# rubengooj/stvo-pl

Hardware: AMD Instinct MI355X
Metric: stereo frames/s (match+optimizePose) (higher is better)
Workload: dtype u8/fp4+f64; 1 GPU; BASELINE configs[2]: KITTI-00-shaped stereo with points + lines (ORB + LBD rows), grid-windowed stereo match (points and lines) + f2f brute-force mutual-NNR match (points and lines) + full GN optimizePose (config_kitti.yaml), device-resident per-frame pipeline; the streams cycle through the 8 sequence ids / 3 KITTI calibrations of configs[4] (sequence s on rank s mod G); streams_per_gpu=3072, parallelism=seq-shard x1

## Files before the change

stvo-pl_amd/csrc/grid_kernels.hip:

```cpp
#include <cstdlib>
#include <vector>

#include "ctx_internal.h"
#include "point_cells.h"

namespace stvo {
namespace {

#ifndef GRID_ROWS_PER_TRIP
#define GRID_ROWS_PER_TRIP 1
#endif
constexpr unsigned long long kTop2Empty = 0x00000000FFFFFFFFull;

struct GridArgs {
    const int32_t* cell_xy1;
    const uint8_t* d1;
    int n1;
    const int32_t* cell_start;
    const int32_t* cell_items;
    const uint8_t* d2;
    int n2;
    const double* dir2;
    stvo_grid_window w;
    double ratio, line_sim_th;
    int mutual;
    int words64;
    int n1p;
    unsigned long long* cover;
    const int32_t* rank;
    const int32_t* perm;
    unsigned long long* top2;
    int32_t* owner2;
    int32_t* m12;
    uint32_t* elig;
    int32_t* elig_cnt;
    int32_t* ovf;
    int elig_stride;
    const int32_t* range1;
};

__device__ __forceinline__ GridArgs frame_view(const GridBatch& g, int b) {
    GridArgs a;
    a.cell_xy1 = g.cell_xy1 + (size_t)b * g.stride1 * g.xy_width;
    a.d1 = g.d1 + (size_t)b * g.stride1 * STVO_DESC_BYTES;
    a.n1 = g.n1[b];
    a.cell_start = g.cell_start + (size_t)b * (STVO_GRID_CELLS + 1);
    a.cell_items = g.cell_items + (size_t)b * g.items_stride;
    a.d2 = g.d2 + (size_t)b * g.stride2 * STVO_DESC_BYTES;
    a.n2 = g.n2[b];
    a.dir2 = g.dir2 ? g.dir2 + (size_t)b * g.stride2 * 2 : nullptr;
    a.w = g.w;
    a.ratio = g.ratio;
    a.line_sim_th = g.line_sim_th;
    a.mutual = g.mutual;
    a.words64 = g.words64;
    a.n1p = g.n1p;
    a.cover = g.cover + (size_t)b * g.words64 * g.n1p;
    a.rank = g.rank + (size_t)b * g.stride2;
    a.perm = g.perm + (size_t)b * g.stride2;
    a.top2 = g.top2 + (size_t)b * g.stride1;
    a.owner2 = g.owner2 + (size_t)b * g.stride2;
    a.m12 = g.m12 + (size_t)b * g.stride1;
    a.elig = g.elig ? g.elig + (size_t)b * GRID_ELIG * g.stride2 : nullptr;
    a.elig_cnt = g.elig ? g.elig_cnt + (size_t)b * g.stride2 : nullptr;
    a.ovf = g.elig ? g.ovf + b : nullptr;
    a.elig_stride = g.stride2;
    a.range1 = g.range1 ? g.range1 + (size_t)b * g.stride1 * 2 : nullptr;
    return a;
}

template <typename P>
__device__ __forceinline__ void cover_window(const GridArgs& a, int x, int y, P col, size_t stride) {
    const int min_x = max(0, x - a.w.w_lo), max_x = min(STVO_GRID_COLS, x + a.w.w_hi + 1);
    const int min_y = max(0, y - a.w.h_lo), max_y = min(STVO_GRID_ROWS, y + a.w.h_hi + 1);
    for (int yy = min_y; yy < max_y; ++yy) {
        if (min_x >= max_x) break;
        const int lo = a.cell_start[yy * STVO_GRID_COLS + min_x], hi = a.cell_start[yy * STVO_GRID_COLS + max_x];
        for (int k = lo; k < hi; ++k) {
            const int id = a.cell_items[k];
            if (id >= 0 && id < a.n2) {
                const int p = a.rank[id];
                col[(size_t)(p >> 6) * stride] |= 1ull << (p & 63);
            }
        }
// ... 220 lines not shown
    }
}

__global__ __launch_bounds__(256) void grid_elig_kernel(GridBatch g) {
    grid_elig_body(frame_view(g, blockIdx.y), blockIdx.x * 256 + threadIdx.x);
}

__device__ __forceinline__ void grid_finalize_body(const GridArgs& a, const int i1, const int stride1) {
    if (i1 >= stride1) return;
    if (i1 >= a.n1) {
        a.m12[i1] = -1;
        return;
    }
    const unsigned long long t = a.top2[i1];
    const uint32_t b = (uint32_t)t, blocked = (uint32_t)(t >> 32);
    int m = -1;
    if (b != 0xFFFFFFFFu && !blocked && (double)(int)(b >> 16) < 2147483647.0 * a.ratio) m = (int)(b & 0xFFFFu);
    if (a.mutual && m >= 0 && a.owner2[m] != i1) m = -1;
    a.m12[i1] = m;
}

__global__ __launch_bounds__(256) void grid_finalize_kernel(GridBatch g) {
    grid_finalize_body(frame_view(g, blockIdx.y), blockIdx.x * 256 + threadIdx.x, g.stride1);
}

constexpr int FUSED_T = 1024, FUSED_ROWS = 2048, FUSED_REG = 16, FUSED_R = FUSED_ROWS / FUSED_T;
constexpr int FUSED_LW = GRID_LW;
constexpr int FUSED_PADDED = FUSED_ROWS + FUSED_REG;
constexpr int FUSED_KEY_CAP = 8192;
constexpr int FUSED_WQ = 256, FUSED_WQ_WORDS = 12;
constexpr size_t FUSED_LDS = (size_t)FUSED_PADDED * (16 + 16 + 2) + (size_t)FUSED_ROWS * (4 + 2 + 2 + 1) + (size_t)FUSED_KEY_CAP * 4 +
                             (size_t)FUSED_WQ * FUSED_WQ_WORDS * 4;

__device__ __forceinline__ void fused_misfit_frame(const GridBatch& g, const int f) {
    const GridArgs a = frame_view(g, f);
    const int stride1 = g.stride1;
    const int tid = threadIdx.x, lane = tid & 63, wave = tid >> 6;
    const int blocks = (a.n2 + 63) >> 6;
    if (g.lean_cells) {
        const int32_t* cs = g.cell_start + (size_t)f * (STVO_GRID_CELLS + 1);
        const uint32_t* ls = g.lstart + (size_t)f * GRID_LSTART_STRIDE;
        const int32_t* lp = g.lperm + (size_t)f * g.stride1;
        int32_t* rg = const_cast<int32_t*>(g.range1) + (size_t)f * g.stride1 * 2;
        for (int i = tid; i < stride1; i += FUSED_T) {
            a.top2[i] = kTop2Empty;
            rg[2 * i] = 0;
            rg[2 * i + 1] = 0;
        }
        if (tid == 0 && a.ovf) *a.ovf = 0;
        __builtin_amdgcn_fence(__ATOMIC_RELEASE, "agent");
        __syncthreads();
        __builtin_amdgcn_fence(__ATOMIC_ACQUIRE, "agent");
        const int n_in = cs[STVO_GRID_CELLS];
        for (int c = tid; c < GRID_LCELLS; c += FUSED_T) {
            const int y = c / GRID_LW, x = c - y * GRID_LW;
            const int min_x = min(max(0, x - g.w.w_lo), STVO_GRID_COLS), max_x = max(min(STVO_GRID_COLS, x + 1), min_x);
            const int c0 = y * STVO_GRID_COLS + min_x, c1 = y * STVO_GRID_COLS + max_x;
            const int lo = c0 < STVO_GRID_CELLS ? cs[c0] : n_in, hi = c1 < STVO_GRID_CELLS ? cs[c1] : n_in;
            for (uint32_t pos = ls[c]; pos < ls[c + 1]; ++pos) {
                const int i1 = lp[pos];
                rg[2 * i1] = lo;
                rg[2 * i1 + 1] = hi;
            }
        }
        __builtin_amdgcn_fence(__ATOMIC_RELEASE, "agent");
        __syncthreads();
        __builtin_amdgcn_fence(__ATOMIC_ACQUIRE, "agent");
    }
    for (int w = wave; w < blocks; w += FUSED_T / 64) grid_scan_body<false, 1, true>(a, w * 64 + lane);
    __builtin_amdgcn_fence(__ATOMIC_RELEASE, "agent");
    __syncthreads();
    __builtin_amdgcn_fence(__ATOMIC_ACQUIRE, "agent");
    if (a.elig)
        for (int w = wave; w < blocks; w += FUSED_T / 64) grid_elig_body(a, w * 64 + lane);
    for (int w = wave; w < blocks; w += FUSED_T / 64) grid_scan_body<false, 2, true>(a, w * 64 + lane);
    __builtin_amdgcn_fence(__ATOMIC_RELEASE, "agent");
    __syncthreads();
    __builtin_amdgcn_fence(__ATOMIC_ACQUIRE, "agent");
    for (int i1 = tid; i1 < stride1; i1 += FUSED_T) grid_finalize_body(a, i1, stride1);
}

typedef uint32_t u32x4 __attribute__((ext_vector_type(4)));
__device__ __forceinline__ uint4 lds_row(const uint4* p) {
    const u32x4 v = *reinterpret_cast<const u32x4*>(p);
    return make_uint4(v.x, v.y, v.z, v.w);
}

__device__ __forceinline__ uint32_t hamming256(const uint4& t0, const uint4& t1, const uint4& q0, const uint4& q1) {
    uint32_t dd = __builtin_popcount(t0.x ^ q0.x);
    dd = bcnt_acc(t0.y ^ q0.y, dd);
    dd = bcnt_acc(t0.z ^ q0.z, dd);
    dd = bcnt_acc(t0.w ^ q0.w, dd);
    dd = bcnt_acc(t1.x ^ q1.x, dd);
    dd = bcnt_acc(t1.y ^ q1.y, dd);
    dd = bcnt_acc(t1.z ^ q1.z, dd);
    dd = bcnt_acc(t1.w ^ q1.w, dd);
    return dd;
}

__device__ __forceinline__ void sort16(uint32_t (&k)[FUSED_REG]) {
#pragma unroll
    for (int size = 2; size <= FUSED_REG; size <<= 1) {
#pragma unroll
        for (int j = size >> 1; j > 0; j >>= 1) {
#pragma unroll
            for (int i = 0; i < FUSED_REG; ++i) {
                const int l = i ^ j;
                if (l > i) {
                    const uint32_t lo = min(k[i], k[l]), hi = max(k[i], k[l]);
                    const bool asc = (i & size) == 0;
                    k[i] = asc ? lo : hi;
                    k[l] = asc ? hi : lo;
                }
            }
        }
    }
}

constexpr int FUSED_EK = 4;
constexpr uint32_t FUSED_NOKEY = 0xFFFFFFFFu, FUSED_FLAG = 1u << 30;

struct FusedNext {
    int i1[FUSED_R], i2[FUSED_R], rc[FUSED_R];
    u32x4 l0[FUSED_R], l1[FUSED_R];
    u32x4 q0[FUSED_R], q1[FUSED_R];
    int la[FUSED_R], lb[FUSED_R];
};

struct FusedHdr {
    int n_placed, n2, n1;
};
__device__ __forceinline__ FusedHdr fused_hdr(const GridBatch& g, const int f) {
    FusedHdr h;
    h.n_placed = (int)g.lstart[(size_t)f * GRID_LSTART_STRIDE + GRID_LCELLS];
    h.n2 = g.n2[f];
    h.n1 = g.n1[f];
    return h;
}

__device__ __forceinline__ int fresh(int v) {
    asm volatile("" : "+v"(v));
    return v;
}

__device__ __forceinline__ void fused_fetch1(const GridBatch& g, const int f, FusedNext& n) {
    const int tid = fresh(threadIdx.x);
    const int32_t* __restrict__ cell2 = g.cell2 + (size_t)f * g.stride2;
    const int32_t* __restrict__ lperm = g.lperm + (size_t)f * g.stride1;
    const int32_t* __restrict__ perm = g.perm + (size_t)f * g.stride2;
#pragma unroll
    for (int r = 0; r < FUSED_R; ++r) {
        const int pos = tid + r * FUSED_T;
        const int p1 = pos < g.stride1 ? pos : g.stride1 - 1, p2 = pos < g.stride2 ? pos : g.stride2 - 1;
        n.i1[r] = lperm[p1];
        n.i2[r] = perm[p2];
        n.rc[r] = cell2[p2];
    }
}

__device__ __forceinline__ void fused_fetch2(const GridBatch& g, const int f, const FusedHdr& h, FusedNext& n) {
    const int tid = fresh(threadIdx.x);
    const u32x4* __restrict__ D1 = reinterpret_cast<const u32x4*>(g.d1) + (size_t)f * g.stride1 * 2;
    const u32x4* __restrict__ D2 = reinterpret_cast<const u32x4*>(g.d2) + (size_t)f * g.stride2 * 2;
    const uint32_t* __restrict__ lstart = g.lstart + (size_t)f * GRID_LSTART_STRIDE;
#pragma unroll
    for (int r = 0; r < FUSED_R; ++r) {
        const int pos = tid + r * FUSED_T;
        const int i1 = pos < h.n_placed ? n.i1[r] : 0, i2 = pos < h.n2 ? n.i2[r] : 0, rc = pos < h.n2 ? n.rc[r] : 0;
        n.l0[r] = D1[2 * i1];
        n.l1[r] = D1[2 * i1 + 1];
        n.q0[r] = D2[2 * i2];
        n.q1[r] = D2[2 * i2 + 1];
        const int y = rc >> 6, x = rc & (STVO_GRID_COLS - 1);
        n.la[r] = (int)lstart[y * FUSED_LW + x];
        n.lb[r] = (int)lstart[y * FUSED_LW + x + g.w.w_lo + 1];
    }
}

__device__ __forceinline__ void fused_tail(const GridBatch& g, const int f, const int n1, const int (&mm)[FUSED_R], int* s_cnt) {
    const PointTail& t = g.tail;
    int tid = threadIdx.x;
    asm volatile("" : "+v"(tid));
    const int lane = tid & 63, wv = tid >> 6;
    const size_t off = (size_t)f * g.stride1;
    bool ok[FUSED_R];
    double disp[FUSED_R];
    int before[FUSED_R];
#pragma unroll
    for (int r = 0; r < FUSED_R; ++r) {
        const int i = tid + r * FUSED_T;
        ok[r] = false;
        disp[r] = 0.0;
        if (i < n1 && mm[r] >= 0) ok[r] = point_tail_filter(t, off, i, mm[r], disp[r]);
        const unsigned long long bal = __ballot(ok[r]);
        before[r] = __popcll(bal & ((1ull << lane) - 1ull));
        if (lane == 0) s_cnt[r * (FUSED_T / 64) + wv] = __popcll(bal);
    }
    __syncthreads();
    int base = 0;
#pragma unroll
    for (int r = 0; r < FUSED_R; ++r) {
        int wbase = base;
        for (int w = 0; w < FUSED_T / 64; ++w) {
            const int c = s_cnt[r * (FUSED_T / 64) + w];
            wbase += w < wv ? c : 0;
            base += c;
        }
        if (ok[r]) point_tail_write(t, off, tid + r * FUSED_T, off + (size_t)(wbase + before[r]), disp[r]);
    }
    if (tid == 0) {
        t.n[f] = base;
        if (t.host_n) t.host_n[f] = base;
        if (t.zero_nl) t.nl[f] = 0;
    }
}

template <bool CELLS>
__global__ __launch_bounds__(FUSED_T) void grid_points_fused_kernel(GridBatch g, const int key_cap) {
    extern __shared__ uint4 s_fused[];
    static_assert(sizeof(PointCellsLds<FUSED_T>) <= FUSED_LDS, "the cells phase borrows the matcher's LDS");
    if (CELLS) {
        if ((int)blockIdx.x >= g.B) return;
        point_cells_frame<FUSED_T, true>(g.cells, blockIdx.x, reinterpret_cast<PointCellsLds<FUSED_T>*>(s_fused));
        __builtin_amdgcn_fence(__ATOMIC_RELEASE, "agent");
        __syncthreads();
        __builtin_amdgcn_fence(__ATOMIC_ACQUIRE, "agent");
    }
    __shared__ int s_cnt[FUSED_R * (FUSED_T / 64)];
    __shared__ int s_ctl[3];
    uint4* s_llo = s_fused;
    uint4* s_lhi = s_llo + FUSED_PADDED;
    uint32_t* s_best = reinterpret_cast<uint32_t*>(s_lhi + FUSED_PADDED);
    uint32_t* s_keys = s_best + FUSED_ROWS;
    unsigned short* s_lperm = reinterpret_cast<unsigned short*>(s_keys + FUSED_KEY_CAP);
    unsigned short* s_owner = s_lperm + FUSED_PADDED;
    unsigned short* s_rperm = s_owner + FUSED_ROWS;
    unsigned char* s_blocked = reinterpret_cast<unsigned char*>(s_rperm + FUSED_ROWS);
    uint32_t* s_wq = reinterpret_cast<uint32_t*>(s_blocked + FUSED_ROWS);
    const int tid = threadIdx.x;
    FusedNext nx;
    int f = blockIdx.x, f_n1 = f + (int)gridDim.x, f_n2 = f + 2 * (int)gridDim.x;
    if (f >= g.B) return;
    unsigned long long misfit_mask = 0ull;
    int trip = 0;
    FusedHdr hn = fused_hdr(g, f);
    fused_fetch1(g, f, nx);
    FusedHdr hc;
    hc.n_placed = __builtin_amdgcn_readfirstlane(hn.n_placed);
    hc.n2 = __builtin_amdgcn_readfirstlane(hn.n2);
    hc.n1 = __builtin_amdgcn_readfirstlane(hn.n1);
    fused_fetch2(g, f, hc, nx);
    if (f_n1 < g.B) hn = fused_hdr(g, f_n1);
    const bool mutual = g.mutual != 0;
    const double ratio = g.ratio;
    FusedHdr hs = hc;
    auto commit_rows = [&](const FusedHdr& h) {
        const int t0 = fresh(tid);
#pragma unroll
        for (int r = 0; r < FUSED_R; ++r) {
            const int pos = t0 + r * FUSED_T;
            if (pos < h.n_placed) {
                *reinterpret_cast<u32x4*>(s_llo + pos) = nx.l0[r];
                *reinterpret_cast<u32x4*>(s_lhi + pos) = nx.l1[r];
                s_lperm[pos] = (unsigned short)nx.i1[r];
            }
        }
        hs.n_placed = __builtin_amdgcn_readfirstlane(hn.n_placed);
        hs.n2 = __builtin_amdgcn_readfirstlane(hn.n2);
        hs.n1 = __builtin_amdgcn_readfirstlane(hn.n1);
    };
    commit_rows(hc);
    for (; f < g.B; f = f_n1, f_n1 = f_n2, f_n2 += (int)gridDim.x) {
        uint4 q0[FUSED_R], q1[FUSED_R];
        int la[FUSED_R], cnt[FUSED_R];
        const int t1 = fresh(tid);
#pragma unroll
        for (int r = 0; r < FUSED_R; ++r) {
            const int pos = t1 + r * FUSED_T;
            if (pos < hc.n2) s_rperm[pos] = (unsigned short)nx.i2[r];
            s_best[pos] = 0xFFFFFFFFu;
            s_blocked[pos] = 0;
            q0[r] = make_uint4(nx.q0[r].x, nx.q0[r].y, nx.q0[r].z, nx.q0[r].w);
            q1[r] = make_uint4(nx.q1[r].x, nx.q1[r].y, nx.q1[r].z, nx.q1[r].w);
            la[r] = pos < hc.n2 ? nx.la[r] : 0;
            cnt[r] = pos < hc.n2 ? nx.lb[r] - nx.la[r] : 0;
        }
        if (tid == 0) {
            s_ctl[0] = 0;
            s_ctl[1] = key_cap < 0;
            s_ctl[2] = 0;
        }
        const int fn = f_n1;
        const bool more = fn < g.B;
        if (more) {
            fused_fetch1(g, fn, nx);
            if (f_n2 < g.B) hn = fused_hdr(g, f_n2);
        }
        __syncthreads();
        uint32_t ek[FUSED_R][FUSED_EK];
        uint32_t kinfo[FUSED_R] = {};
#pragma unroll
        for (int r = 0; r < FUSED_R; ++r) {
            const int p = tid + r * FUSED_T;
            uint32_t key[FUSED_REG];
            uint32_t elig = 0u;
            bool wide = cnt[r] > FUSED_REG;
            if (wide) {
                const int xoff = atomicAdd(&s_ctl[0], cnt[r]);
                const int slot = atomicAdd(&s_ctl[2], 1);
                if (xoff + cnt[r] > key_cap || slot >= FUSED_WQ) {
                    s_ctl[1] = 1;
                    wide = false;
                    cnt[r] = 0;
                } else {
                    kinfo[r] = (uint32_t)cnt[r] | ((uint32_t)xoff << 12) | 0x80000000u;
                    uint32_t* e = s_wq + slot * FUSED_WQ_WORDS;
                    e[0] = (uint32_t)p; e[1] = (uint32_t)la[r]; e[2] = (uint32_t)cnt[r]; e[3] = (uint32_t)xoff;
                    e[4] = q0[r].x; e[5] = q0[r].y; e[6] = q0[r].z; e[7] = q0[r].w;
                    e[8] = q1[r].x; e[9] = q1[r].y; e[10] = q1[r].z; e[11] = q1[r].w;
                }
            }
            const int c16 = wide ? 0 : cnt[r];
            const uint4* lo_row = s_llo + la[r];
            const uint4* hi_row = s_lhi + la[r];
            const unsigned short* perm_row = s_lperm + la[r];
#pragma unroll
            for (int k4 = 0; k4 < FUSED_REG; k4 += 4) {
                if (!__any(c16 > k4)) {
#pragma unroll
                    for (int j = 0; j < 4; ++j) key[k4 + j] = FUSED_NOKEY;
                    continue;
                }
#pragma unroll
                for (int j = 0; j < 4; ++j) {
                    const uint32_t dd = hamming256(lds_row(lo_row + k4 + j), lds_row(hi_row + k4 + j), q0[r], q1[r]);
                    const uint32_t i1 = perm_row[k4 + j];
                    key[k4 + j] = k4 + j < c16 ? ((i1 << 9) | dd) : FUSED_NOKEY;
                }
            }
            uint32_t owner = 0xFFFFu;
            if (mutual) {
                sort16(key);
                uint32_t thr = 512u;
#pragma unroll
                for (int k = 0; k < FUSED_REG; ++k) {
                    const uint32_t dd = key[k] & 511u;
                    if (key[k] != FUSED_NOKEY && dd < thr) {
                        thr = dd;
                        owner = key[k] >> 9;
                        elig |= 1u << k;
                    }
                }
            } else {
                elig = (1u << c16) - 1u;
            }
            int extra = __builtin_popcount(elig) - FUSED_EK, eoff = 0;
            if (extra > 0) {
                eoff = atomicAdd(&s_ctl[0], extra);
                if (eoff + extra > key_cap) {
                    s_ctl[1] = 1;
                    extra = 0;
                } else {
                    kinfo[r] = (uint32_t)extra | ((uint32_t)eoff << 12);
                }
            }
#pragma unroll
            for (int j = 0; j < FUSED_EK; ++j) ek[r][j] = FUSED_NOKEY;
            int ne = 0;
#pragma unroll
            for (int k = 0; k < FUSED_REG; ++k)
                if (elig & (1u << k)) {
                    atomicMin(&s_best[key[k] >> 9], ((key[k] & 511u) << 16) | (uint32_t)p);
#pragma unroll
                    for (int j = 0; j < FUSED_EK; ++j) ek[r][j] = ne == j ? key[k] : ek[r][j];
                    if (k >= FUSED_EK && ne >= FUSED_EK && ne - FUSED_EK < extra) s_keys[eoff + ne - FUSED_EK] = key[k];
                    ++ne;
                }
            if (!wide) s_owner[p] = (unsigned short)owner;
            if (wide && !mutual) s_owner[p] = 0xFFFFu;
        }
        if (more) fused_fetch2(g, fn, hs, nx);
        __syncthreads();
        const bool misfit = s_ctl[1] != 0;
        const int n_wide = s_ctl[2];
        if (!misfit && n_wide > 0) {
            for (int ent = tid >> 6; ent < n_wide; ent += FUSED_T / 64) {
                const uint32_t* e = s_wq + ent * FUSED_WQ_WORDS;
                const uint32_t w_p = (uint32_t)__builtin_amdgcn_readfirstlane((int)e[0]);
                const int w_la = __builtin_amdgcn_readfirstlane((int)e[1]), w_cnt = __builtin_amdgcn_readfirstlane((int)e[2]);
                const int w_xoff = __builtin_amdgcn_readfirstlane((int)e[3]);
                const uint4 wq0 = make_uint4(e[4], e[5], e[6], e[7]), wq1 = make_uint4(e[8], e[9], e[10], e[11]);
                uint32_t* kk = s_keys + w_xoff;
                for (int k = tid & 63; k < w_cnt; k += 64) {
                    const int pos = w_la + k;
                    kk[k] = ((uint32_t)s_lperm[pos] << 9) | hamming256(lds_row(s_llo + pos), lds_row(s_lhi + pos), wq0, wq1);
                }
                __builtin_amdgcn_fence(__ATOMIC_RELEASE, "wavefront");
                __builtin_amdgcn_wave_barrier();
                __builtin_amdgcn_fence(__ATOMIC_ACQUIRE, "wavefront");
                for (int k = tid & 63; k < w_cnt; k += 64) {
                    const uint32_t mine = kk[k] & ~FUSED_FLAG, i1 = mine >> 9, dd = mine & 511u;
                    bool dominated = false, later_better = false;
                    for (int j = 0; j < w_cnt; ++j) {
                        const uint32_t v = kk[j], vi = (v >> 9) & 2047u, vd = v & 511u;
                        dominated |= vi < i1 && vd <= dd;
                        later_better |= vi > i1 && vd < dd;
                    }
                    if (!mutual || !dominated) {
                        kk[k] = mine | FUSED_FLAG;
                        atomicMin(&s_best[i1], (dd << 16) | w_p);
                        if (mutual && !later_better) s_owner[w_p] = (unsigned short)i1;
                    }
                }
            }
            __syncthreads();
        }
        if (tid == 0) g.misfit[f] = misfit;
        if (misfit && trip < 64) misfit_mask |= 1ull << trip;
        ++trip;
        if (!misfit) {
#pragma unroll
            for (int r = 0; r < FUSED_R; ++r) {
                const uint32_t p = (uint32_t)(tid + r * FUSED_T);
                auto judge = [&](uint32_t k, uint32_t pos) {
                    const uint32_t i1 = (k >> 9) & 2047u, dd = k & 511u;
                    const uint32_t bk = s_best[i1];
                    if (bk != ((dd << 16) | pos)) {
                        const double best_d = (double)(int)(bk >> 16), d2 = (double)(int)dd;
                        if (!(best_d < d2 * ratio)) s_blocked[i1] = 1;
                    }
                };
#pragma unroll
                for (int j = 0; j < FUSED_EK; ++j)
                    if (ek[r][j] != FUSED_NOKEY) judge(ek[r][j], p);
                if (!(kinfo[r] >> 31))
                    for (uint32_t j = 0; j < (kinfo[r] & 4095u); ++j) judge(s_keys[((kinfo[r] >> 12) & 0x3FFFFu) + j], p);
                for (unsigned long long wm = __ballot((kinfo[r] >> 31) != 0u); wm; wm &= wm - 1ull) {
                    const int L = __builtin_ctzll(wm);
                    const uint32_t w_info = (uint32_t)__builtin_amdgcn_readlane((int)kinfo[r], L);
                    const int w_cnt = (int)(w_info & 4095u), w_xoff = (int)((w_info >> 12) & 0x3FFFFu);
                    const uint32_t w_p = (uint32_t)((tid & ~63) + L + r * FUSED_T);
                    for (int k = tid & 63; k < w_cnt; k += 64) {
                        const uint32_t v = s_keys[w_xoff + k];
                        if (v & FUSED_FLAG) judge(v & ~FUSED_FLAG, w_p);
                    }
                }
            }
        }
        const FusedHdr hfn = hs;
        if (more) commit_rows(hfn);
        __syncthreads();
        if (!misfit) {
            int mm[FUSED_R];
#pragma unroll
            for (int r = 0; r < FUSED_R; ++r) {
                const int i1 = tid + r * FUSED_T;
                mm[r] = -1;
                if (i1 >= g.stride1) continue;
                const uint32_t bk = s_best[i1];
                if (i1 < hc.n1 && bk != 0xFFFFFFFFu && !s_blocked[i1] && (double)(int)(bk >> 16) < 2147483647.0 * ratio) {
                    const int pb = (int)(bk & 0xFFFFu);
                    if (!mutual || (int)s_owner[pb] == i1) mm[r] = (int)s_rperm[pb];
                }
                g.m12[(size_t)f * g.stride1 + i1] = mm[r];
            }
            if (g.has_tail) fused_tail(g, f, hc.n1, mm, s_cnt);
        }
        if (more) __syncthreads();
        hc = hfn;
    }
    if (misfit_mask != 0ull || trip > 64) {
        int i = 0;
        for (int fm = (int)blockIdx.x; fm < g.B; fm += (int)gridDim.x, ++i) {
            const bool todo = i < 64 ? ((misfit_mask >> i) & 1ull) != 0ull : g.misfit[fm] != 0;
            if (todo) {
                __syncthreads();
                fused_misfit_frame(g, fm);
                if (g.has_tail) {
                    __builtin_amdgcn_fence(__ATOMIC_RELEASE, "agent");
                    __syncthreads();
                    __builtin_amdgcn_fence(__ATOMIC_ACQUIRE, "agent");
                    int mm[FUSED_R];
#pragma unroll
                    for (int r = 0; r < FUSED_R; ++r) {
                        const int i1 = threadIdx.x + r * FUSED_T;
                        mm[r] = i1 < g.stride1 ? g.m12[(size_t)fm * g.stride1 + i1] : -1;
                    }
                    fused_tail(g, fm, g.n1[fm], mm, s_cnt);
                }
            }
        }
    }
}

}

bool grid_points_fused_ok(const GridBatch& g) {
    const bool range = g.range_points && g.range1 != nullptr;
    const bool fused = range && g.misfit && g.cell2 && g.lperm && g.lstart && g.stride1 <= FUSED_ROWS && g.stride2 <= FUSED_ROWS && g.w.w_lo >= 0 &&
                       g.w.w_lo <= FUSED_LW - STVO_GRID_COLS && g.w.w_hi == 0 && g.w.h_lo == 0 && g.w.h_hi == 0 && dbg().grid_fused != 0;
    return fused && lds_opt_in(reinterpret_cast<const void*>(grid_points_fused_kernel<false>), (int)FUSED_LDS) &&
           lds_opt_in(reinterpret_cast<const void*>(grid_points_fused_kernel<true>), (int)FUSED_LDS);
}

void launch_grid_batch(hipStream_t s, const GridBatch& g, bool lines, hipEvent_t* scan_events) {
    if (g.B <= 0 || g.stride1 <= 0 || g.stride2 <= 0) return;
    const dim3 g1((g.stride1 + 255) / 256, g.B), g2((g.stride2 + 255) / 256, g.B), gc((g.n1p + 255) / 256, g.B), blk(256);
    const size_t lds = (size_t)g.words64 * 256 * sizeof(unsigned long long);
    const bool use_lds = lds <= ((size_t)64 << 10);
    if (lines) {
        if (use_lds)
            hipLaunchKernelGGL((grid_cover_kernel<true, true>), gc, blk, lds, s, g);
        else
            hipLaunchKernelGGL((grid_cover_kernel<true, false>), gc, blk, 0, s, g);
        if (scan_events && scan_events[0]) (void)hipEventRecord(scan_events[0], s);
        hipLaunchKernelGGL((grid_scan_kernel<true, 1, false>), g2, blk, 0, s, g);
        if (g.elig) hipLaunchKernelGGL(grid_elig_kernel, g2, blk, 0, s, g);
        hipLaunchKernelGGL((grid_scan_kernel<true, 2, false>), g2, blk, 0, s, g);
        if (scan_events) (void)hipEventRecord(scan_events[1], s);
    } else {
        const bool range = g.range_points && g.range1 != nullptr;
        if (grid_points_fused_ok(g)) {
            int cap = dbg().grid_fused_cap != DBG_UNSET ? dbg().grid_fused_cap : FUSED_KEY_CAP;
            if (cap > FUSED_KEY_CAP) cap = FUSED_KEY_CAP;
            const int fused_wgs = device_cu_count();
            if (scan_events && scan_events[0]) (void)hipEventRecord(scan_events[0], s);
            if (g.fused_cells && g.B <= fused_wgs)
                hipLaunchKernelGGL(grid_points_fused_kernel<true>, dim3(g.B), dim3(FUSED_T), FUSED_LDS, s, g, cap);
            else
                hipLaunchKernelGGL(grid_points_fused_kernel<false>, dim3(g.B < fused_wgs ? g.B : fused_wgs), dim3(FUSED_T), FUSED_LDS, s, g, cap);
            if (scan_events) (void)hipEventRecord(scan_events[1], s);
            return;
        }
        if (range) {
            if (scan_events && scan_events[0]) (void)hipEventRecord(scan_events[0], s);
            hipLaunchKernelGGL((grid_scan_kernel<false, 1, true>), g2, blk, 0, s, g);
            if (g.elig) hipLaunchKernelGGL(grid_elig_kernel, g2, blk, 0, s, g);
            hipLaunchKernelGGL((grid_scan_kernel<false, 2, true>), g2, blk, 0, s, g);
        } else {
            if (use_lds)
                hipLaunchKernelGGL((grid_cover_kernel<false, true>), gc, blk, lds, s, g);
            else
                hipLaunchKernelGGL((grid_cover_kernel<false, false>), gc, blk, 0, s, g);
            if (scan_events && scan_events[0]) (void)hipEventRecord(scan_events[0], s);
            hipLaunchKernelGGL((grid_scan_kernel<false, 1, false>), g2, blk, 0, s, g);
            if (g.elig) hipLaunchKernelGGL(grid_elig_kernel, g2, blk, 0, s, g);
            hipLaunchKernelGGL((grid_scan_kernel<false, 2, false>), g2, blk, 0, s, g);
        }
        if (scan_events) (void)hipEventRecord(scan_events[1], s);
    }
    hipLaunchKernelGGL(grid_finalize_kernel, g1, blk, 0, s, g);
}

void launch_grid_range_debug(hipStream_t s, const GridBatch& g) {
    hipLaunchKernelGGL(grid_range_debug_kernel, dim3((g.n1p + 255) / 256, g.B), dim3(256), 0, s, g);
}

namespace {

template <bool LINES>
int run_grid(stvo_ctx* ctx, const int32_t* cell_xy1, const uint8_t* d1, int n1, const int32_t* cell_start,
             const int32_t* cell_items, const uint8_t* d2, int n2, const double* dir2, const stvo_grid_window* w,
             double ratio, double line_sim_th, int mutual, int32_t* m12, int32_t* n_matches) {
// ... 117 lines not shown
```

stvo-pl_amd/csrc/match_mfma.hip:

```cpp
#include <type_traits>

#include "kernels.h"

namespace stvo {

typedef int v4i __attribute__((ext_vector_type(4)));
typedef int v8i __attribute__((ext_vector_type(8)));
typedef int v16i __attribute__((ext_vector_type(16)));
typedef float v16f __attribute__((ext_vector_type(16)));

#ifndef MF_TPB
#define MF_TPB 2
#endif
#ifndef MF_FOLD_SLOTS
#define MF_FOLD_SLOTS 5
#endif
constexpr int MF_BLOCK = 256;
constexpr int MF_TILE = 32;
constexpr int MF_KEY_SHIFT = 13;
constexpr int MF_KEY_BIAS = 1 << 20;
constexpr int MF_NO_KEY = 0x7FFFFFFF;
constexpr int MF_NO_KEY_MIN = 0x40000000;

__device__ __forceinline__ v4i expand_fp4(uint32_t w) {
    v4i r;
    r.x = (int)(((w << 3) & 0x88888888u) | 0x66666666u);
    r.y = (int)(((w << 2) & 0x88888888u) | 0x66666666u);
    r.z = (int)(((w << 1) & 0x88888888u) | 0x66666666u);
    r.w = (int)((w & 0x88888888u) | 0x66666666u);
    return r;
}
__device__ __forceinline__ float med3_f32(float a, float b, float c) {
    float r;
    asm("v_med3_f32 %0, %1, %2, %3" : "=v"(r) : "v"(a), "v"(b), "v"(c));
    return r;
}
__device__ __forceinline__ float min_f32(float a, float b) {
    float r;
    asm("v_min_f32 %0, %1, %2" : "=v"(r) : "v"(a), "v"(b));
    return r;
}
__device__ __forceinline__ float max_f32(float a, float b) {
    float r;
    asm("v_max_f32 %0, %1, %2" : "=v"(r) : "v"(a), "v"(b));
    return r;
}
__device__ __forceinline__ float min3_f32(float a, float b, float c) {
    float r;
    asm("v_min3_f32 %0, %1, %2, %3" : "=v"(r) : "v"(a), "v"(b), "v"(c));
    return r;
}
constexpr float MF_NO_KEY_F = 1.0e30f;
constexpr float MF_NO_KEY_MIN_F = 1.0e29f;
constexpr int MF_SCALE_2_4 = 127 + 4;

__device__ __forceinline__ uint32_t key_to_knn(int key, int base) {
    if (key >= MF_NO_KEY_MIN) return 0xFFFFFFFFu;
    const uint32_t u = (uint32_t)(key + base + MF_KEY_BIAS);
    return ((u >> MF_KEY_SHIFT) << 16) | (u & ((1u << MF_KEY_SHIFT) - 1u));
}

template <int QB, int MODE>
// ... 461 lines not shown
```

stvo-pl_amd/csrc/point_tail.h:

```cpp
#pragma once

#include <hip/hip_runtime.h>
#include <stdint.h>

#include "../../include/stvo_hip.h"

namespace stvo {

struct PointTail {
    const float* kp_l;
    const float* kp_r;
    const int32_t* oct_l;
    const uint8_t* desc_l;
    const stvo_cam* cams;
    double max_dist_epip, min_disp;
    float4* rc;
    uint8_t* desc;
    int32_t* n;
    int32_t* host_n;
    int32_t* nl;
    int zero_nl;
};

__device__ __forceinline__ bool point_tail_filter(const PointTail& t, size_t off, int i, int i2, double& disp) {
    const float yl = t.kp_l[(off + i) * 2 + 1], yr = t.kp_r[(off + i2) * 2 + 1];
    if (!((double)fabsf(yl - yr) <= t.max_dist_epip)) return false;
    disp = (double)(t.kp_l[(off + i) * 2 + 0] - t.kp_r[(off + i2) * 2 + 0]);
    return disp >= t.min_disp;
}

__device__ __forceinline__ void point_tail_write(const PointTail& t, size_t off, int i, size_t k, double disp) {
    t.rc[k] = make_float4(t.kp_l[(off + i) * 2 + 0], t.kp_l[(off + i) * 2 + 1], (float)disp, (float)t.oct_l[off + i]);
    const uint4* src = reinterpret_cast<const uint4*>(t.desc_l + (off + i) * STVO_DESC_BYTES);
    uint4* dst = reinterpret_cast<uint4*>(t.desc + k * STVO_DESC_BYTES);
    dst[0] = src[0];
    dst[1] = src[1];
}

}
```

Measured before the change: 1.380 million frame-pairs/s.

## Read fused grid kernel args from kernarg segment and tighten inner-loop instructions

The fused point grid matcher now reads GridBatch fields through the kernarg segment pointer on each use instead of holding a by-value copy, aiming to cut scalar register pressure. The Hamming key building folds the i1<<9 term into the popcount accumulator and masks invalid slots with a bit-field sign extract instead of a select. The eligible-key buffering becomes a shift register, and the tail prefetches left keypoints, batches right-keypoint loads and computes disparity in float. The fp4 expansion uses a single and-or instruction, and an optional cycle-counter probe, compiled out by default, is added.

```diff
diff --git a/stvo-pl_amd/csrc/grid_kernels.hip b/stvo-pl_amd/csrc/grid_kernels.hip
--- a/stvo-pl_amd/csrc/grid_kernels.hip
+++ b/stvo-pl_amd/csrc/grid_kernels.hip
@@ -1,3 +1,4 @@
+#include <cstdio>
 #include <cstdlib>
 #include <vector>
 
@@ -39,7 +40,8 @@
     const int32_t* range1;
 };
 
-__device__ __forceinline__ GridArgs frame_view(const GridBatch& g, int b) {
+template <class G>
+__device__ __forceinline__ GridArgs frame_view(const G& g, int b) {
     GridArgs a;
     a.cell_xy1 = g.cell_xy1 + (size_t)b * g.stride1 * g.xy_width;
     a.d1 = g.d1 + (size_t)b * g.stride1 * STVO_DESC_BYTES;
@@ -49,7 +51,7 @@
     a.d2 = g.d2 + (size_t)b * g.stride2 * STVO_DESC_BYTES;
     a.n2 = g.n2[b];
     a.dir2 = g.dir2 ? g.dir2 + (size_t)b * g.stride2 * 2 : nullptr;
-    a.w = g.w;
+    a.w.w_lo = g.w.w_lo; a.w.w_hi = g.w.w_hi; a.w.h_lo = g.w.h_lo; a.w.h_hi = g.w.h_hi;
     a.ratio = g.ratio;
     a.line_sim_th = g.line_sim_th;
     a.mutual = g.mutual;
@@ -336,7 +338,9 @@
 constexpr size_t FUSED_LDS = (size_t)FUSED_PADDED * (16 + 16 + 2) + (size_t)FUSED_ROWS * (4 + 2 + 2 + 1) + (size_t)FUSED_KEY_CAP * 4 +
                              (size_t)FUSED_WQ * FUSED_WQ_WORDS * 4;
 
-__device__ __forceinline__ void fused_misfit_frame(const GridBatch& g, const int f) {
+template <class KA>
+__device__ __forceinline__ void fused_misfit_frame(KA ka, const int f) {
+    const auto& g = ka();
     const GridArgs a = frame_view(g, f);
     const int stride1 = g.stride1;
     const int tid = threadIdx.x, lane = tid & 63, wave = tid >> 6;
@@ -358,7 +362,7 @@
         const int n_in = cs[STVO_GRID_CELLS];
         for (int c = tid; c < GRID_LCELLS; c += FUSED_T) {
             const int y = c / GRID_LW, x = c - y * GRID_LW;
-            const int min_x = min(max(0, x - g.w.w_lo), STVO_GRID_COLS), max_x = max(min(STVO_GRID_COLS, x + 1), min_x);
+            const int min_x = min(max(0, x - a.w.w_lo), STVO_GRID_COLS), max_x = max(min(STVO_GRID_COLS, x + 1), min_x);
             const int c0 = y * STVO_GRID_COLS + min_x, c1 = y * STVO_GRID_COLS + max_x;
             const int lo = c0 < STVO_GRID_CELLS ? cs[c0] : n_in, hi = c1 < STVO_GRID_CELLS ? cs[c1] : n_in;
             for (uint32_t pos = ls[c]; pos < ls[c + 1]; ++pos) {
@@ -390,8 +394,8 @@
     return make_uint4(v.x, v.y, v.z, v.w);
 }
 
-__device__ __forceinline__ uint32_t hamming256(const uint4& t0, const uint4& t1, const uint4& q0, const uint4& q1) {
-    uint32_t dd = __builtin_popcount(t0.x ^ q0.x);
+__device__ __forceinline__ uint32_t hamming256(const uint4& t0, const uint4& t1, const uint4& q0, const uint4& q1, const uint32_t init = 0u) {
+    uint32_t dd = bcnt_acc(t0.x ^ q0.x, init);
     dd = bcnt_acc(t0.y ^ q0.y, dd);
     dd = bcnt_acc(t0.z ^ q0.z, dd);
     dd = bcnt_acc(t0.w ^ q0.w, dd);
@@ -402,6 +406,12 @@
     return dd;
 }
 
+__device__ __forceinline__ uint32_t sign_of_bit(const uint32_t x, const int bit) {
+    int r;
+    asm("v_bfe_i32 %0, %1, %2, 1" : "=v"(r) : "v"(x), "n"(bit));
+    return (uint32_t)r;
+}
+
 __device__ __forceinline__ void sort16(uint32_t (&k)[FUSED_REG]) {
 #pragma unroll
     for (int size = 2; size <= FUSED_REG; size <<= 1) {
@@ -434,7 +444,10 @@
 struct FusedHdr {
     int n_placed, n2, n1;
 };
-__device__ __forceinline__ FusedHdr fused_hdr(const GridBatch& g, const int f) {
+typedef const GridBatch __attribute__((address_space(4))) FusedKArgs;
+template <class KA>
+__device__ __forceinline__ FusedHdr fused_hdr(KA ka, const int f) {
+    const auto& g = ka();
     FusedHdr h;
     h.n_placed = (int)g.lstart[(size_t)f * GRID_LSTART_STRIDE + GRID_LCELLS];
     h.n2 = g.n2[f];
@@ -447,26 +460,32 @@
     return v;
 }
 
-__device__ __forceinline__ void fused_fetch1(const GridBatch& g, const int f, FusedNext& n) {
+template <class KA>
+__device__ __forceinline__ void fused_fetch1(KA ka, const int f, FusedNext& n) {
+    const auto& g = ka();
     const int tid = fresh(threadIdx.x);
     const int32_t* __restrict__ cell2 = g.cell2 + (size_t)f * g.stride2;
     const int32_t* __restrict__ lperm = g.lperm + (size_t)f * g.stride1;
     const int32_t* __restrict__ perm = g.perm + (size_t)f * g.stride2;
+    const int stride1 = g.stride1, stride2 = g.stride2;
 #pragma unroll
     for (int r = 0; r < FUSED_R; ++r) {
         const int pos = tid + r * FUSED_T;
-        const int p1 = pos < g.stride1 ? pos : g.stride1 - 1, p2 = pos < g.stride2 ? pos : g.stride2 - 1;
+        const int p1 = pos < stride1 ? pos : stride1 - 1, p2 = pos < stride2 ? pos : stride2 - 1;
         n.i1[r] = lperm[p1];
         n.i2[r] = perm[p2];
         n.rc[r] = cell2[p2];
     }
 }
 
-__device__ __forceinline__ void fused_fetch2(const GridBatch& g, const int f, const FusedHdr& h, FusedNext& n) {
+template <class KA>
+__device__ __forceinline__ void fused_fetch2(KA ka, const int f, const FusedHdr& h, FusedNext& n) {
+    const auto& g = ka();
     const int tid = fresh(threadIdx.x);
     const u32x4* __restrict__ D1 = reinterpret_cast<const u32x4*>(g.d1) + (size_t)f * g.stride1 * 2;
     const u32x4* __restrict__ D2 = reinterpret_cast<const u32x4*>(g.d2) + (size_t)f * g.stride2 * 2;
     const uint32_t* __restrict__ lstart = g.lstart + (size_t)f * GRID_LSTART_STRIDE;
+    const int w_lo = g.w.w_lo;
 #pragma unroll
     for (int r = 0; r < FUSED_R; ++r) {
         const int pos = tid + r * FUSED_T;
@@ -477,30 +496,99 @@
         n.q1[r] = D2[2 * i2 + 1];
         const int y = rc >> 6, x = rc & (STVO_GRID_COLS - 1);
         n.la[r] = (int)lstart[y * FUSED_LW + x];
-        n.lb[r] = (int)lstart[y * FUSED_LW + x + g.w.w_lo + 1];
-    }
-}
-
-__device__ __forceinline__ void fused_tail(const GridBatch& g, const int f, const int n1, const int (&mm)[FUSED_R], int* s_cnt) {
-    const PointTail& t = g.tail;
-    int tid = threadIdx.x;
-    asm volatile("" : "+v"(tid));
-    const int lane = tid & 63, wv = tid >> 6;
-    const size_t off = (size_t)f * g.stride1;
-    bool ok[FUSED_R];
-    double disp[FUSED_R];
-    int before[FUSED_R];
+        n.lb[r] = (int)lstart[y * FUSED_LW + x + w_lo + 1];
+    }
+}
+
+#ifdef STVO_GRID_PROBE
+constexpr bool kFusedProbe = true;
+#else
+constexpr bool kFusedProbe = false;
+#endif
+constexpr int FUSED_NPH = 16;
+enum FusedPhase { PH_COMMIT = 0, PH_W_COMMIT, PH_DIST, PH_W_DIST, PH_WIDE, PH_W_WIDE, PH_RATIO, PH_ROWS_WAIT, PH_ROWS, PH_W_ROWS, PH_ACCEPT, PH_W_TAIL,
+                  PH_WRITE, PH_W_END };
+template <bool PROF>
+struct FusedTicks {
+    uint32_t acc[FUSED_NPH];
+    long long last;
+    __device__ __forceinline__ void start() {
+        if constexpr (PROF) {
+#pragma unroll
+            for (int i = 0; i < FUSED_NPH; ++i) acc[i] = 0u;
+            last = (long long)__builtin_readcyclecounter();
+        }
+    }
+    __device__ __forceinline__ void operator()(const int slot) {
+        if constexpr (PROF) {
+            const long long t = (long long)__builtin_readcyclecounter();
+            acc[slot] += (uint32_t)(t - last);
+            last = t;
+        }
+    }
+    __device__ __forceinline__ void flush(uint32_t* out, const int f) {
+        if constexpr (PROF) {
+            if ((threadIdx.x & 63) == 0) {
+                uint32_t* o = out + ((size_t)f * (FUSED_T / 64) + (threadIdx.x >> 6)) * FUSED_NPH;
+#pragma unroll
+                for (int i = 0; i < FUSED_NPH; ++i) o[i] = acc[i];
+            }
+#pragma unroll
+            for (int i = 0; i < FUSED_NPH; ++i) acc[i] = 0u;
+        }
+    }
+};
+
+template <class KA>
+__device__ __forceinline__ void fused_tail_fetch(KA ka, const int f, float2 (&kl)[FUSED_R]) {
+    const auto& g = ka();
+    const int tid = fresh(threadIdx.x);
+    const int stride1 = g.stride1;
+    const float2* __restrict__ kp_l = reinterpret_cast<const float2*>(g.tail.kp_l) + (size_t)f * stride1;
 #pragma unroll
     for (int r = 0; r < FUSED_R; ++r) {
         const int i = tid + r * FUSED_T;
-        ok[r] = false;
-        disp[r] = 0.0;
-        if (i < n1 && mm[r] >= 0) ok[r] = point_tail_filter(t, off, i, mm[r], disp[r]);
-        const unsigned long long bal = __ballot(ok[r]);
-        before[r] = __popcll(bal & ((1ull << lane) - 1ull));
-        if (lane == 0) s_cnt[r * (FUSED_T / 64) + wv] = __popcll(bal);
-    }
+        kl[r] = kp_l[i < stride1 ? i : stride1 - 1];
+    }
+}
+
+template <class KA, class Ticks>
+__device__ __forceinline__ void fused_tail(KA ka, const int f, const int n1, const int (&mm)[FUSED_R], const float2 (&kl)[FUSED_R], int* s_cnt,
+                                           Ticks& tick) {
+    const int tid = fresh(threadIdx.x);
+    const int lane = tid & 63, wv = tid >> 6;
+    bool ok[FUSED_R];
+    float disp[FUSED_R];
+    int before[FUSED_R], oct[FUSED_R];
+    {
+        const auto& g = ka();
+        const size_t off = (size_t)f * g.stride1;
+        const float2* __restrict__ kp_r = reinterpret_cast<const float2*>(g.tail.kp_r) + off;
+        const int32_t* __restrict__ oct_l = g.tail.oct_l + off;
+        const double max_dist_epip = g.tail.max_dist_epip, min_disp = g.tail.min_disp;
+        float2 kr[FUSED_R];
+#pragma unroll
+        for (int r = 0; r < FUSED_R; ++r) kr[r] = kp_r[mm[r] >= 0 ? mm[r] : 0];
+#pragma unroll
+        for (int r = 0; r < FUSED_R; ++r) {
+            const int i = tid + r * FUSED_T;
+            double d = 0.0;
+            ok[r] = i < n1 && mm[r] >= 0 && point_tail_pass(kl[r].x, kl[r].y, kr[r].x, kr[r].y, max_dist_epip, min_disp, d);
+            disp[r] = (float)d;
+            const unsigned long long bal = __ballot(ok[r]);
+            before[r] = __popcll(bal & ((1ull << lane) - 1ull));
+            if (lane == 0) s_cnt[r * (FUSED_T / 64) + wv] = __popcll(bal);
+            if (ok[r]) oct[r] = oct_l[i];
+        }
+    }
+    tick(PH_ACCEPT);
     __syncthreads();
+    tick(PH_W_TAIL);
+    const auto& g = ka();
+    const size_t off = (size_t)f * g.stride1;
+    float4* __restrict__ rc = g.tail.rc + off;
+    const u32x4* __restrict__ desc_l = reinterpret_cast<const u32x4*>(g.tail.desc_l) + off * 2;
+    u32x4* __restrict__ desc = reinterpret_cast<u32x4*>(g.tail.desc) + off * 2;
     int base = 0;
 #pragma unroll
     for (int r = 0; r < FUSED_R; ++r) {
@@ -510,19 +598,32 @@
             wbase += w < wv ? c : 0;
             base += c;
         }
-        if (ok[r]) point_tail_write(t, off, tid + r * FUSED_T, off + (size_t)(wbase + before[r]), disp[r]);
+        if (ok[r]) {
+            const int k = wbase + before[r];
+            const int i = tid + r * FUSED_T;
+            const u32x4 d0 = desc_l[2 * i], d1 = desc_l[2 * i + 1];
+            rc[k] = make_float4(kl[r].x, kl[r].y, disp[r], (float)oct[r]);
+            desc[2 * k] = d0;
+            desc[2 * k + 1] = d1;
+        }
     }
     if (tid == 0) {
-        t.n[f] = base;
-        if (t.host_n) t.host_n[f] = base;
-        if (t.zero_nl) t.nl[f] = 0;
-    }
-}
-
-template <bool CELLS>
-__global__ __launch_bounds__(FUSED_T) void grid_points_fused_kernel(GridBatch g, const int key_cap) {
+        g.tail.n[f] = base;
+        if (g.tail.host_n) g.tail.host_n[f] = base;
+        if (g.tail.zero_nl) g.tail.nl[f] = 0;
+    }
+}
+
+template <bool CELLS, bool PROF>
+__global__ __launch_bounds__(FUSED_T) void grid_points_fused_kernel(GridBatch g, const int key_cap, uint32_t* const prof_out) {
     extern __shared__ uint4 s_fused[];
     static_assert(sizeof(PointCellsLds<FUSED_T>) <= FUSED_LDS, "the cells phase borrows the matcher's LDS");
+    FusedKArgs* const kargs = (FusedKArgs*)__builtin_amdgcn_kernarg_segment_ptr();
+    auto ka = [&]() -> FusedKArgs& {
+        FusedKArgs* p = kargs;
+        asm volatile("" : "+s"(p));
+        return *p;
+    };
     if (CELLS) {
         if ((int)blockIdx.x >= g.B) return;
         point_cells_frame<FUSED_T, true>(g.cells, blockIdx.x, reinterpret_cast<PointCellsLds<FUSED_T>*>(s_fused));
@@ -544,19 +645,20 @@
     const int tid = threadIdx.x;
     FusedNext nx;
     int f = blockIdx.x, f_n1 = f + (int)gridDim.x, f_n2 = f + 2 * (int)gridDim.x;
-    if (f >= g.B) return;
+    const int B = ka().B;
+    if (f >= B) return;
     unsigned long long misfit_mask = 0ull;
     int trip = 0;
-    FusedHdr hn = fused_hdr(g, f);
-    fused_fetch1(g, f, nx);
+    FusedHdr hn = fused_hdr(ka, f);
+    fused_fetch1(ka, f, nx);
     FusedHdr hc;
     hc.n_placed = __builtin_amdgcn_readfirstlane(hn.n_placed);
     hc.n2 = __builtin_amdgcn_readfirstlane(hn.n2);
     hc.n1 = __builtin_amdgcn_readfirstlane(hn.n1);
-    fused_fetch2(g, f, hc, nx);
-    if (f_n1 < g.B) hn = fused_hdr(g, f_n1);
-    const bool mutual = g.mutual != 0;
-    const double ratio = g.ratio;
+    fused_fetch2(ka, f, hc, nx);
+    if (f_n1 < B) hn = fused_hdr(ka, f_n1);
+    const bool mutual = ka().mutual != 0;
+    const double ratio = ka().ratio;
     FusedHdr hs = hc;
     auto commit_rows = [&](const FusedHdr& h) {
         const int t0 = fresh(tid);
@@ -574,7 +676,9 @@
         hs.n1 = __builtin_amdgcn_readfirstlane(hn.n1);
     };
     commit_rows(hc);
-    for (; f < g.B; f = f_n1, f_n1 = f_n2, f_n2 += (int)gridDim.x) {
+    FusedTicks<PROF> tick;
+    tick.start();
+    for (; f < B; f = f_n1, f_n1 = f_n2, f_n2 += (int)gridDim.x) {
         uint4 q0[FUSED_R], q1[FUSED_R];
         int la[FUSED_R], cnt[FUSED_R];
         const int t1 = fresh(tid);
@@ -595,12 +699,14 @@
             s_ctl[2] = 0;
         }
         const int fn = f_n1;
-        const bool more = fn < g.B;
+        const bool more = fn < B;
         if (more) {
-            fused_fetch1(g, fn, nx);
-            if (f_n2 < g.B) hn = fused_hdr(g, f_n2);
-        }
+            fused_fetch1(ka, fn, nx);
+            if (f_n2 < B) hn = fused_hdr(ka, f_n2);
+        }
+        tick(PH_COMMIT);
         __syncthreads();
+        tick(PH_W_COMMIT);
         uint32_t ek[FUSED_R][FUSED_EK];
         uint32_t kinfo[FUSED_R] = {};
 #pragma unroll
@@ -628,6 +734,7 @@
             const uint4* lo_row = s_llo + la[r];
             const uint4* hi_row = s_lhi + la[r];
             const unsigned short* perm_row = s_lperm + la[r];
+            const uint32_t past = ~((1u << c16) - 1u);
 #pragma unroll
             for (int k4 = 0; k4 < FUSED_REG; k4 += 4) {
                 if (!__any(c16 > k4)) {
@@ -637,9 +744,9 @@
                 }
 #pragma unroll
                 for (int j = 0; j < 4; ++j) {
-                    const uint32_t dd = hamming256(lds_row(lo_row + k4 + j), lds_row(hi_row + k4 + j), q0[r], q1[r]);
                     const uint32_t i1 = perm_row[k4 + j];
-                    key[k4 + j] = k4 + j < c16 ? ((i1 << 9) | dd) : FUSED_NOKEY;
+                    const uint32_t kd = hamming256(lds_row(lo_row + k4 + j), lds_row(hi_row + k4 + j), q0[r], q1[r], i1 << 9);
+                    key[k4 + j] = kd | sign_of_bit(past, k4 + j);
                 }
             }
             uint32_t owner = 0xFFFFu;
@@ -670,21 +777,23 @@
             }
 #pragma unroll
             for (int j = 0; j < FUSED_EK; ++j) ek[r][j] = FUSED_NOKEY;
-            int ne = 0;
+            int nev = 0;
 #pragma unroll
             for (int k = 0; k < FUSED_REG; ++k)
                 if (elig & (1u << k)) {
                     atomicMin(&s_best[key[k] >> 9], ((key[k] & 511u) << 16) | (uint32_t)p);
-#pragma unroll
-                    for (int j = 0; j < FUSED_EK; ++j) ek[r][j] = ne == j ? key[k] : ek[r][j];
-                    if (k >= FUSED_EK && ne >= FUSED_EK && ne - FUSED_EK < extra) s_keys[eoff + ne - FUSED_EK] = key[k];
-                    ++ne;
+                    if (k >= FUSED_EK && extra > 0 && ek[r][0] != FUSED_NOKEY) s_keys[eoff + nev++] = ek[r][0];
+#pragma unroll
+                    for (int j = 0; j + 1 < FUSED_EK; ++j) ek[r][j] = ek[r][j + 1];
+                    ek[r][FUSED_EK - 1] = key[k];
                 }
             if (!wide) s_owner[p] = (unsigned short)owner;
             if (wide && !mutual) s_owner[p] = 0xFFFFu;
         }
-        if (more) fused_fetch2(g, fn, hs, nx);
+        if (more) fused_fetch2(ka, fn, hs, nx);
+        tick(PH_DIST);
         __syncthreads();
+        tick(PH_W_DIST);
         const bool misfit = s_ctl[1] != 0;
         const int n_wide = s_ctl[2];
         if (!misfit && n_wide > 0) {
@@ -697,7 +806,7 @@
                 uint32_t* kk = s_keys + w_xoff;
                 for (int k = tid & 63; k < w_cnt; k += 64) {
                     const int pos = w_la + k;
-                    kk[k] = ((uint32_t)s_lperm[pos] << 9) | hamming256(lds_row(s_llo + pos), lds_row(s_lhi + pos), wq0, wq1);
+                    kk[k] = hamming256(lds_row(s_llo + pos), lds_row(s_lhi + pos), wq0, wq1, (uint32_t)s_lperm[pos] << 9);
                 }
                 __builtin_amdgcn_fence(__ATOMIC_RELEASE, "wavefront");
                 __builtin_amdgcn_wave_barrier();
@@ -717,9 +826,11 @@
                     }
                 }
             }
+            tick(PH_WIDE);
             __syncthreads();
-        }
-        if (tid == 0) g.misfit[f] = misfit;
+            tick(PH_W_WIDE);
+        }
+        if (tid == 0) ka().misfit[f] = misfit;
         if (misfit && trip < 64) misfit_mask |= 1ull << trip;
         ++trip;
         if (!misfit) {
@@ -752,35 +863,53 @@
             }
         }
         const FusedHdr hfn = hs;
+        tick(PH_RATIO);
+        if (PROF && more) {
+            asm volatile("s_waitcnt vmcnt(0)" ::: "memory");
+            tick(PH_ROWS_WAIT);
+        }
         if (more) commit_rows(hfn);
+        const bool has_tail = ka().has_tail != 0;
+        float2 kl[FUSED_R];
+        if (!misfit && has_tail) fused_tail_fetch(ka, f, kl);
+        tick(PH_ROWS);
         __syncthreads();
+        tick(PH_W_ROWS);
         if (!misfit) {
             int mm[FUSED_R];
 #pragma unroll
             for (int r = 0; r < FUSED_R; ++r) {
                 const int i1 = tid + r * FUSED_T;
                 mm[r] = -1;
-                if (i1 >= g.stride1) continue;
                 const uint32_t bk = s_best[i1];
                 if (i1 < hc.n1 && bk != 0xFFFFFFFFu && !s_blocked[i1] && (double)(int)(bk >> 16) < 2147483647.0 * ratio) {
                     const int pb = (int)(bk & 0xFFFFu);
                     if (!mutual || (int)s_owner[pb] == i1) mm[r] = (int)s_rperm[pb];
                 }
-                g.m12[(size_t)f * g.stride1 + i1] = mm[r];
-            }
-            if (g.has_tail) fused_tail(g, f, hc.n1, mm, s_cnt);
-        }
+            }
+            if (has_tail) fused_tail(ka, f, hc.n1, mm, kl, s_cnt, tick);
+            const int stride1 = ka().stride1;
+            int32_t* __restrict__ m12 = ka().m12 + (size_t)f * stride1;
+#pragma unroll
+            for (int r = 0; r < FUSED_R; ++r) {
+                const int i1 = fresh(tid) + r * FUSED_T;
+                if (i1 < stride1) m12[i1] = mm[r];
+            }
+        }
+        tick(PH_WRITE);
         if (more) __syncthreads();
+        tick(PH_W_END);
+        tick.flush(prof_out, f);
         hc = hfn;
     }
     if (misfit_mask != 0ull || trip > 64) {
         int i = 0;
-        for (int fm = (int)blockIdx.x; fm < g.B; fm += (int)gridDim.x, ++i) {
-            const bool todo = i < 64 ? ((misfit_mask >> i) & 1ull) != 0ull : g.misfit[fm] != 0;
+        for (int fm = (int)blockIdx.x; fm < B; fm += (int)gridDim.x, ++i) {
+            const bool todo = i < 64 ? ((misfit_mask >> i) & 1ull) != 0ull : ka().misfit[fm] != 0;
             if (todo) {
                 __syncthreads();
-                fused_misfit_frame(g, fm);
-                if (g.has_tail) {
+                fused_misfit_frame(ka, fm);
+                if (ka().has_tail) {
                     __builtin_amdgcn_fence(__ATOMIC_RELEASE, "agent");
                     __syncthreads();
                     __builtin_amdgcn_fence(__ATOMIC_ACQUIRE, "agent");
@@ -788,23 +917,57 @@
 #pragma unroll
                     for (int r = 0; r < FUSED_R; ++r) {
                         const int i1 = threadIdx.x + r * FUSED_T;
-                        mm[r] = i1 < g.stride1 ? g.m12[(size_t)fm * g.stride1 + i1] : -1;
+                        mm[r] = i1 < ka().stride1 ? ka().m12[(size_t)fm * ka().stride1 + i1] : -1;
                     }
-                    fused_tail(g, fm, g.n1[fm], mm, s_cnt);
-                }
-            }
-        }
-    }
-}
-
+                    float2 kl[FUSED_R];
+                    fused_tail_fetch(ka, fm, kl);
+                    fused_tail(ka, fm, ka().n1[fm], mm, kl, s_cnt, tick);
+                }
+            }
+        }
+    }
+}
+
+}
+
+namespace {
+uint32_t* fused_probe_buffer(hipStream_t s, const int B) {
+    static uint32_t* buf = nullptr;
+    static int cap = 0;
+    if (B > cap) {
+        if (buf) (void)hipFree(buf);
+        buf = nullptr;
+        cap = 0;
+        if (hipMalloc(reinterpret_cast<void**>(&buf), (size_t)B * (FUSED_T / 64) * FUSED_NPH * sizeof(uint32_t)) == hipSuccess) cap = B;
+    }
+    if (buf) (void)hipMemsetAsync(buf, 0, (size_t)B * (FUSED_T / 64) * FUSED_NPH * sizeof(uint32_t), s);
+    return buf;
+}
+void fused_probe_report(hipStream_t s, const int B, const bool cells, const uint32_t* prof) {
+    static const char* const names[FUSED_NPH] = {"commit", "w_commit", "distance", "w_distance", "wide", "w_wide", "ratio", "rows_wait", "rows_commit",
+                                                 "w_rows", "accept_filter", "w_tail", "tail_write", "w_end", "-", "-"};
+    static int launch = 0;
+    if (!prof || hipStreamSynchronize(s) != hipSuccess) return;
+    std::vector<uint32_t> h((size_t)B * (FUSED_T / 64) * FUSED_NPH);
+    if (hipMemcpy(h.data(), prof, h.size() * sizeof(uint32_t), hipMemcpyDeviceToHost) != hipSuccess) return;
+    double sum[FUSED_NPH] = {}, total = 0.0;
+    for (size_t i = 0; i < h.size(); ++i) sum[i % FUSED_NPH] += (double)h[i];
+    const double n = (double)B * (FUSED_T / 64);
+    std::fprintf(stderr, "grid_probe launch %d B %d cells %d cycles per frame and wave:", launch++, B, (int)cells);
+    for (int i = 0; i < PH_W_END + 1; ++i) {
+        std::fprintf(stderr, " %s %.0f", names[i], sum[i] / n);
+        total += sum[i] / n;
+    }
+    std::fprintf(stderr, " total %.0f\n", total);
+}
 }
 
 bool grid_points_fused_ok(const GridBatch& g) {
     const bool range = g.range_points && g.range1 != nullptr;
     const bool fused = range && g.misfit && g.cell2 && g.lperm && g.lstart && g.stride1 <= FUSED_ROWS && g.stride2 <= FUSED_ROWS && g.w.w_lo >= 0 &&
                        g.w.w_lo <= FUSED_LW - STVO_GRID_COLS && g.w.w_hi == 0 && g.w.h_lo == 0 && g.w.h_hi == 0 && dbg().grid_fused != 0;
-    return fused && lds_opt_in(reinterpret_cast<const void*>(grid_points_fused_kernel<false>), (int)FUSED_LDS) &&
-           lds_opt_in(reinterpret_cast<const void*>(grid_points_fused_kernel<true>), (int)FUSED_LDS);
+    return fused && lds_opt_in(reinterpret_cast<const void*>(grid_points_fused_kernel<false, kFusedProbe>), (int)FUSED_LDS) &&
+           lds_opt_in(reinterpret_cast<const void*>(grid_points_fused_kernel<true, kFusedProbe>), (int)FUSED_LDS);
 }
 
 void launch_grid_batch(hipStream_t s, const GridBatch& g, bool lines, hipEvent_t* scan_events) {
@@ -829,10 +992,14 @@
             if (cap > FUSED_KEY_CAP) cap = FUSED_KEY_CAP;
             const int fused_wgs = device_cu_count();
             if (scan_events && scan_events[0]) (void)hipEventRecord(scan_events[0], s);
-            if (g.fused_cells && g.B <= fused_wgs)
-                hipLaunchKernelGGL(grid_points_fused_kernel<true>, dim3(g.B), dim3(FUSED_T), FUSED_LDS, s, g, cap);
+            const bool cells = g.fused_cells && g.B <= fused_wgs;
+            uint32_t* const prof = kFusedProbe ? fused_probe_buffer(s, g.B) : nullptr;
+            if (cells)
+                hipLaunchKernelGGL((grid_points_fused_kernel<true, kFusedProbe>), dim3(g.B), dim3(FUSED_T), FUSED_LDS, s, g, cap, prof);
             else
-                hipLaunchKernelGGL(grid_points_fused_kernel<false>, dim3(g.B < fused_wgs ? g.B : fused_wgs), dim3(FUSED_T), FUSED_LDS, s, g, cap);
+                hipLaunchKernelGGL((grid_points_fused_kernel<false, kFusedProbe>), dim3(g.B < fused_wgs ? g.B : fused_wgs), dim3(FUSED_T), FUSED_LDS, s,
+                                   g, cap, prof);
+            if (kFusedProbe) fused_probe_report(s, g.B, cells, prof);
             if (scan_events) (void)hipEventRecord(scan_events[1], s);
             return;
         }
diff --git a/stvo-pl_amd/csrc/match_mfma.hip b/stvo-pl_amd/csrc/match_mfma.hip
--- a/stvo-pl_amd/csrc/match_mfma.hip
+++ b/stvo-pl_amd/csrc/match_mfma.hip
@@ -22,12 +22,17 @@
 constexpr int MF_NO_KEY = 0x7FFFFFFF;
 constexpr int MF_NO_KEY_MIN = 0x40000000;
 
+__device__ __forceinline__ int fp4_nibbles(uint32_t x) {
+    int r;
+    asm("v_and_or_b32 %0, %1, %2, %3" : "=v"(r) : "v"(x), "s"(0x88888888u), "v"(0x66666666u));
+    return r;
+}
 __device__ __forceinline__ v4i expand_fp4(uint32_t w) {
     v4i r;
-    r.x = (int)(((w << 3) & 0x88888888u) | 0x66666666u);
-    r.y = (int)(((w << 2) & 0x88888888u) | 0x66666666u);
-    r.z = (int)(((w << 1) & 0x88888888u) | 0x66666666u);
-    r.w = (int)((w & 0x88888888u) | 0x66666666u);
+    r.x = fp4_nibbles(w << 3);
+    r.y = fp4_nibbles(w << 2);
+    r.z = fp4_nibbles(w << 1);
+    r.w = fp4_nibbles(w);
     return r;
 }
 __device__ __forceinline__ float med3_f32(float a, float b, float c) {
diff --git a/stvo-pl_amd/csrc/point_tail.h b/stvo-pl_amd/csrc/point_tail.h
--- a/stvo-pl_amd/csrc/point_tail.h
+++ b/stvo-pl_amd/csrc/point_tail.h
@@ -22,11 +22,15 @@
     int zero_nl;
 };
 
+__device__ __forceinline__ bool point_tail_pass(float xl, float yl, float xr, float yr, double max_dist_epip, double min_disp, double& disp) {
+    if (!((double)fabsf(yl - yr) <= max_dist_epip)) return false;
+    disp = (double)(xl - xr);
+    return disp >= min_disp;
+}
+
 __device__ __forceinline__ bool point_tail_filter(const PointTail& t, size_t off, int i, int i2, double& disp) {
-    const float yl = t.kp_l[(off + i) * 2 + 1], yr = t.kp_r[(off + i2) * 2 + 1];
-    if (!((double)fabsf(yl - yr) <= t.max_dist_epip)) return false;
-    disp = (double)(t.kp_l[(off + i) * 2 + 0] - t.kp_r[(off + i2) * 2 + 0]);
-    return disp >= t.min_disp;
+    return point_tail_pass(t.kp_l[(off + i) * 2 + 0], t.kp_l[(off + i) * 2 + 1], t.kp_r[(off + i2) * 2 + 0], t.kp_r[(off + i2) * 2 + 1], t.max_dist_epip,
+                           t.min_disp, disp);
 }
 
 __device__ __forceinline__ void point_tail_write(const PointTail& t, size_t off, int i, size_t k, double disp) {
```

After: 1.362 million frame-pairs/s. 0.987x the previous value.
